# PaulMayer123/IMS-Toucan-Prosody-Variance

Hardware: AMD Instinct MI355X
Metric: mel-frames/sec + vocoder RTF @24kHz, batch=32, 1/2/4/8 MI355X (higher is better)
Workload: dtype bf16

## Files before the change

ims-toucan-prosody-variance_amd/csrc/common.h:

```cpp
#pragma once
#include <hip/hip_runtime.h>
#include <stdint.h>
#include <stdio.h>

#include "../../include/toucan_tts.h"

namespace tts {

void set_error(const char* fmt, ...);

#define TTS_CHECK_ARG(cond, ...)   \
  do {                             \
    if (!(cond)) {                 \
      tts::set_error(__VA_ARGS__); \
      return TTS_E_ARG;            \
    }                              \
  } while (0)

inline int launch_status(const char* what) {
  hipError_t e = hipGetLastError();
  if (e != hipSuccess) {
    set_error("%s: %s", what, hipGetErrorString(e));
    return TTS_E_LAUNCH;
  }
  return TTS_OK;
}

inline hipError_t raise_lds_limit(const void* kernel, unsigned long long& mask) {
  int dev = 0;
  (void)hipGetDevice(&dev);
  const unsigned long long bit = 1ull << (dev & 63);
  if (mask & bit) return hipSuccess;
  int room = 160 * 1024;
  hipFuncAttributes attr;
  if (hipFuncGetAttributes(&attr, kernel) == hipSuccess) room -= (int)attr.sharedSizeBytes;
  else (void)hipGetLastError();
  const hipError_t e = hipFuncSetAttribute(kernel, hipFuncAttributeMaxDynamicSharedMemorySize, room);
  if (e == hipSuccess) mask |= bit;
  else (void)hipGetLastError();
  return e;
}

struct WavenetCond {
  const float* g;
  int ld_g;
  const void* wc;
  int wc_n;
  int col0;
  const float* bc;
};
int wavenet_layer_cond(const TtsWavenetDesc& d, const WavenetCond& c, hipStream_t st);

typedef float f32x16 __attribute__((ext_vector_type(16)));
typedef float f32x4 __attribute__((ext_vector_type(4)));
typedef short bf16x8 __attribute__((ext_vector_type(8)));

__device__ __forceinline__ unsigned short f32_to_bf16(float f) {
  const __bf16 b = (__bf16)f;
  return __builtin_bit_cast(unsigned short, b);
}
__device__ __forceinline__ float bf16_to_f32(unsigned short u) { return __builtin_bit_cast(float, (unsigned int)u << 16); }

typedef _Float16 f16x2 __attribute__((ext_vector_type(2)));
typedef _Float16 f16x8 __attribute__((ext_vector_type(8)));
typedef float f32x2 __attribute__((ext_vector_type(2)));
__device__ __forceinline__ unsigned short f32_to_f16(float f) { return __builtin_bit_cast(unsigned short, (_Float16)f); }
__device__ __forceinline__ float f16_to_f32(unsigned short u) { return (float)__builtin_bit_cast(_Float16, u); }
template <bool F16>
__device__ __forceinline__ unsigned short to16(float f) {
  if constexpr (F16) return f32_to_f16(f);
  else return f32_to_bf16(f);
}
template <bool F16>
__device__ __forceinline__ float from16(unsigned short u) {
  if constexpr (F16) return f16_to_f32(u);
  else return bf16_to_f32(u);
}
template <bool F16>
__device__ __forceinline__ unsigned int pack16(float lo, float hi) {
  if constexpr (F16) {
    const f32x2 v = {lo, hi};
    return __builtin_bit_cast(unsigned int, __builtin_convertvector(v, f16x2));
  } else {
    return (unsigned int)f32_to_bf16(lo) | ((unsigned int)f32_to_bf16(hi) << 16);
  }
}
__device__ __forceinline__ float load16(unsigned short u, bool f16) { return f16 ? f16_to_f32(u) : bf16_to_f32(u); }
__device__ __forceinline__ unsigned short store16(float v, bool f16) { return f16 ? f32_to_f16(v) : f32_to_bf16(v); }

template <bool F16>
__device__ __forceinline__ f32x16 mfma16(bf16x8 a, bf16x8 b, f32x16 c) {
  if constexpr (F16) return __builtin_amdgcn_mfma_f32_32x32x16_f16(__builtin_bit_cast(f16x8, a), __builtin_bit_cast(f16x8, b), c, 0, 0, 0);
  else return __builtin_amdgcn_mfma_f32_32x32x16_bf16(a, b, c, 0, 0, 0);
}

#define TTS_GLOAD128(dst_, ptr_) asm volatile("global_load_dwordx4 %0, %1, off" : "=v"(dst_) : "v"(ptr_) : "memory")
#define TTS_GLOAD32(dst_, ptr_) asm volatile("global_load_dword %0, %1, off" : "=v"(dst_) : "v"(ptr_) : "memory")
#define TTS_WAIT_VM(n_) asm volatile("s_waitcnt vmcnt(%0)" ::"n"(n_) : "memory")
#define TTS_PIN(r_) asm volatile("" : "+v"(r_))

__device__ __forceinline__ float sigmoidf_(float v) { return 1.0f / (1.0f + __expf(-v)); }

__device__ __forceinline__ float wave_sum(float v) {
#pragma unroll
  for (int o = 32; o > 0; o >>= 1) v += __shfl_xor(v, o, 64);
  return v;
}

__device__ __forceinline__ float wave_max(float v) {
#pragma unroll
  for (int o = 32; o > 0; o >>= 1) v = fmaxf(v, __shfl_xor(v, o, 64));
  return v;
}

}
```

ims-toucan-prosody-variance_amd/csrc/conv1d_wide.hip:

```cpp
#include "common.h"
#include "conv_epilogue.h"

namespace tts {

namespace {

constexpr int WIDE_BM = 256, WIDE_BN = 256, WIDE_BK = 64, WIDE_THREADS = 512;
constexpr int WIDE_ROW_BYTES = WIDE_BK * 2;
constexpr int WIDE_SLAB_BYTES = WIDE_BK * WIDE_BN * 2;

__host__ __device__ inline int wide_win_rows(int taps, int dil) { return (WIDE_BM + (taps - 1) * dil + 7) & ~7; }
inline size_t wide_lds_bytes(int taps, int dil) {
  return (size_t)2 * wide_win_rows(taps, dil) * WIDE_ROW_BYTES + 2 * WIDE_SLAB_BYTES + 2 * WIDE_BN * sizeof(float);
}

__device__ __forceinline__ void wide_dma16(const void* src, void* lds_wave_base) {
  __builtin_amdgcn_global_load_lds((const void __attribute__((address_space(1)))*)src, (void __attribute__((address_space(3)))*)lds_wave_base, 16, 0, 0);
}

template <bool F16>
__global__ __launch_bounds__(WIDE_THREADS) void conv1d_wide_kernel(const TtsConvDesc d) {
  constexpr int TM = 4, TN = 2;
  extern __shared__ __attribute__((aligned(16))) unsigned char lds_raw[];

  const TtsTile tile = d.tiles[blockIdx.x];
  const int n0 = blockIdx.y * WIDE_BN;
  const int win_rows = wide_win_rows(d.taps, d.dil);
  const int win_bytes = win_rows * WIDE_ROW_BYTES;
  unsigned char* const xs0 = lds_raw;
  unsigned char* const ws0 = lds_raw + 2 * win_bytes;
  float* const eb = reinterpret_cast<float*>(ws0 + 2 * WIDE_SLAB_BYTES);

  const int tid = threadIdx.x;
  const int lane = tid & 63;
  const int wave = __builtin_amdgcn_readfirstlane(tid >> 6);
  const int wm = wave >> 2, wn = wave & 3;
  const int lrow = lane & 31, lk = lane >> 5;

  f32x16 acc[1][TM][TN];
#pragma unroll
  for (int i = 0; i < TM; ++i)
#pragma unroll
    for (int j = 0; j < TN; ++j)
#pragma unroll
      for (int r = 0; r < 16; ++r) acc[0][i][j][r] = 0.0f;

  if (tid < WIDE_BN) {
    const int n = n0 + tid;
    eb[tid] = (d.bias && n < d.cout) ? d.bias[n] : 0.0f;
    eb[WIDE_BN + tid] = 0.0f;
  }

  const bool poly = d.io_flags & TTS_IO_POLYPHASE;
  const int half = d.wn >> 1;
  const int tap_lo = (poly && n0 >= half) ? 1 : 0;
  const int tap_hi = (poly && n0 + WIDE_BN <= half) ? 2 : d.taps;
  const int wc0 = n0 + wn * 64;
  const int skip_tap = !poly ? -1 : (wc0 >= half ? 0 : (wc0 + 64 <= half ? 2 : -1));

  const int row_first = tile.row0 - d.pad_left;
  const bool edge = row_first < tile.seq_begin || row_first + win_rows > tile.seq_end;
  const unsigned short* __restrict__ xh = reinterpret_cast<const unsigned short*>(d.x);
  const unsigned short* __restrict__ W = reinterpret_cast<const unsigned short*>(d.w);
  const int n_chunks = d.cin / WIDE_BK;
  const int n_win_inst = win_rows >> 3;

  auto request_window = [&](int ch) __attribute__((always_inline)) {
    unsigned char* xb = xs0 + (ch & 1) * win_bytes;
    for (int i = wave; i < n_win_inst; i += 8) {
      const int wr = i * 8 + (lane >> 3);
      const int g = (lane & 7) ^ ((wr >> 1) & 7);
      const int gr = row_first + wr;
      const int grc = gr < tile.seq_begin ? tile.seq_begin : (gr >= tile.seq_end ? tile.seq_end - 1 : gr);
      wide_dma16(xh + (size_t)grc * d.ldx + ch * WIDE_BK + g * 8, xb + i * 1024);
    }
  };
  auto zero_window_edges = [&](int ch) __attribute__((always_inline)) {
    unsigned char* xb = xs0 + (ch & 1) * win_bytes;
    for (int i = wave; i < n_win_inst; i += 8) {
      const int gr = row_first + i * 8 + (lane >> 3);
      if (gr < tile.seq_begin || gr >= tile.seq_end) *reinterpret_cast<uint4*>(xb + i * 1024 + lane * 16) = make_uint4(0, 0, 0, 0);
    }
  };
  auto request_weights = [&](int ch, int tap, int buf) __attribute__((always_inline)) {
    unsigned char* wb = ws0 + buf * WIDE_SLAB_BYTES;
#pragma unroll
    for (int q = 0; q < 4; ++q) {
      const int idx = q * 8 + wave;
      const int kb = idx >> 2, part = idx & 3;
      const size_t goff = (((size_t)tap * (d.cin_pad >> 3) + ch * 8 + kb) * d.wn + n0 + part * 64 + lane) * 8;
      wide_dma16(W + goff, wb + idx * 1024);
    }
  };

  request_window(0);
  request_weights(0, tap_lo, 0);
  bool zero_pending = edge;
  int zero_ch = 0;

  int step = 0;
  for (int ch = 0; ch < n_chunks; ++ch) {
    const unsigned char* xb = xs0 + (ch & 1) * win_bytes;
    for (int tap = tap_lo; tap < tap_hi; ++tap, ++step) {
      asm volatile("s_waitcnt vmcnt(0)" ::: "memory");
      if (zero_pending) {
        zero_window_edges(zero_ch);
        zero_pending = false;
      }
      asm volatile("s_waitcnt lgkmcnt(0)\n\ts_barrier" ::: "memory");
      {
        const bool last_tap = tap + 1 == tap_hi;
        const int nch = last_tap ? ch + 1 : ch, ntap = last_tap ? tap_lo : tap + 1;
        if (nch < n_chunks) request_weights(nch, ntap, (step + 1) & 1);
      }
      if (tap == tap_lo && ch + 1 < n_chunks) {
        request_window(ch + 1);
        zero_pending = edge;
        zero_ch = ch + 1;
      }
      if (tap == skip_tap) continue;
      const unsigned char* wb = ws0 + (step & 1) * WIDE_SLAB_BYTES;
      const int r0 = wm * 128 + lrow + tap * d.dil;
#pragma unroll
      for (int ks = 0; ks < 4; ++ks) {
        const int g = ks * 2 + lk;
        bf16x8 a[TM], b[TN];
#pragma unroll
        for (int j = 0; j < TN; ++j) b[j] = *reinterpret_cast<const bf16x8*>(wb + (size_t)(g * WIDE_BN + wn * 64 + j * 32 + lrow) * 16);
#pragma unroll
        for (int i = 0; i < TM; ++i) {
          const int r = r0 + i * 32;
          a[i] = *reinterpret_cast<const bf16x8*>(xb + r * WIDE_ROW_BYTES + ((g ^ ((r >> 1) & 7)) << 4));
        }
#pragma unroll
        for (int i = 0; i < TM; ++i)
#pragma unroll
          for (int j = 0; j < TN; ++j) acc[0][i][j] = mfma16<F16>(b[j], a[i], acc[0][i][j]);
      }
    }
  }
  conv_epilogue_t<TM, TN, 1, false, true>(d, tile, n0, wm, wn, lrow, lk, acc, eb, WIDE_BN);
}

}

const char* conv1d_wide_reject(const TtsConvDesc& d) {
  auto al16 = [](const void* p) { return (reinterpret_cast<uintptr_t>(p) & 15) == 0; };
  if (d.compute != TTS_COMPUTE_BF16 && d.compute != TTS_COMPUTE_F16) return "compute must be bf16 or fp16";
  if (d.mode != TTS_MODE_LINEAR) return "mode must be LINEAR";
  if (!(d.io_flags & TTS_IO_X_BF16) || !(d.io_flags & TTS_IO_Y_BF16) || (d.res && !(d.io_flags & TTS_IO_RES_BF16))) return "x, y and res must be 16-bit tensors";
  if (((d.io_flags & TTS_IO_F16) != 0) != (d.compute == TTS_COMPUTE_F16)) return "the 16-bit tensors must be in the call's own format";
  if (d.pre_act != TTS_PRE_NONE) return "no pre-activation";
  if (d.seqvec || d.preadd || d.aux) return "no seqvec, preadd or aux";
  if (d.cin != d.cin_pad || d.cin % WIDE_BK != 0) return "cin must be unpadded and a multiple of 64";
  if (d.wn % WIDE_BN != 0 || d.cout > d.wn) return "wn must be a multiple of 256";
  if ((d.cout & 3) || (d.bias && !al16(d.bias))) return "cout must be a multiple of 4 and the bias 16-byte aligned";
  if ((d.ldx & 7) || (d.ldy & 7) || (d.res && (d.ld_res & 7)) || !al16(d.x) || !al16(d.y) || !al16(d.w) || (d.res && !al16(d.res))) return "rows and pointers must be 16-byte aligned";
  if ((d.io_flags & TTS_IO_POLYPHASE) && d.taps != 3) return "TTS_IO_POLYPHASE needs taps == 3";
  if (wide_lds_bytes(d.taps, d.dil) > 160 * 1024) return "the window does not fit in 160 KiB of LDS";
  return nullptr;
}

int conv1d_wide_launch(const TtsConvDesc& d, hipStream_t st) {
  const char* why = conv1d_wide_reject(d);
  TTS_CHECK_ARG(why == nullptr, "conv1d: a 256-row tile table asks for the wide tile, which this call cannot take: %s", why);
  const size_t lds = wide_lds_bytes(d.taps, d.dil);
  dim3 grid(d.n_tiles, d.wn / WIDE_BN), block(WIDE_THREADS);
  auto launch = [&](auto k, unsigned long long& raised) {
    if (lds > 64 * 1024) {
      const hipError_t e = raise_lds_limit(reinterpret_cast<const void*>(k), raised);
      if (e != hipSuccess) {
        set_error("conv1d (wide): raising the dynamic LDS limit failed: %s", hipGetErrorString(e));
        return (int)TTS_E_LAUNCH;
      }
    }
    hipLaunchKernelGGL(k, grid, block, lds, st, d);
    return launch_status("conv1d (wide)");
  };
  static unsigned long long raised_bf16 = 0, raised_f16 = 0;
  if (d.compute == TTS_COMPUTE_F16) return launch(conv1d_wide_kernel<true>, raised_f16);
  return launch(conv1d_wide_kernel<false>, raised_bf16);
}

}
```

ims-toucan-prosody-variance_amd/csrc/pipeline.hip:

```cpp
#include <algorithm>
#include <cmath>
#include <cstdlib>
#include <cstring>
#include <string>
#include <unordered_map>
#include <utility>
#include <vector>

#include "common.h"
#include "../../include/toucan_prosody.h"
#include "../../include/toucan_score.h"

namespace tts {

const char* conv1d_wide_reject(const TtsConvDesc& d);

namespace {

constexpr int ATT = 192, HEADS = 4, DK = 48;

struct Dev {
  void* p = nullptr;
  int64_t shape[4] = {0, 0, 0, 0};
  int ndim = 0, dtype = 0;
// ... 76 lines not shown
  }
  Layout halved() const {
    Layout l;
    for (size_t i = 0; i < begins.size(); ++i) {
      l.begins.push_back(begins[i] / 2);
      l.lengths.push_back(lengths[i] / 2);
      l.max_len = std::max(l.max_len, lengths[i] / 2);
    }
    l.total = total / 2;
    return l;
  }
  int n() const { return (int)lengths.size(); }
};

struct Arena {
  char* base = nullptr;
  size_t cap = 0, off = 0;
  void reset() { off = 0; }
};

struct TileTab {
  TtsTile* dev = nullptr;
  int n = 0;
};

constexpr size_t TABLE_FIRST_CHUNK = 64 << 10;
constexpr size_t TABLE_BUDGET = 16 << 20;

struct TableChunk {
  char* dev = nullptr;
  char* host = nullptr;
  size_t cap = 0, off = 0;
};

struct TableStore {
  std::vector<TableChunk> chunks;
  std::unordered_map<std::string, std::pair<void*, int>> index;
  hipEvent_t last_use = nullptr;
};

struct ProfRec {
  std::string name;
  double flops = 0, bytes = 0, elems = 0;
  hipEvent_t e0 = nullptr, e1 = nullptr;
};

}

struct Handle {
  TtsConfig cfg;
  std::unordered_map<std::string, Dev> weights;
  Acoustic acoustic;
  Vocoder vocoder;
  Arena phone, frame, voc[2];
  Arena nll;
  TableStore tabs[2][2];
  int tab_gen[2] = {0, 0};
  int tab_which = 0;
  long long n_tables_built = 0;
  int small_tile_blocks = 1536;
  int split_mode = 0;
  float* ptab[2] = {nullptr, nullptr};
  int pmax = 0;
  Layout lp, lf;
  int B = 0;
  const float* text = nullptr;
  float *e_norm = nullptr, *enc = nullptr, *pitch = nullptr, *energy = nullptr, *cln = nullptr;
  int* dur = nullptr;
  float *cat = nullptr, *dec = nullptr, *mel0 = nullptr, *mel = nullptr;
  std::vector<int> frames;
  float* pstats = nullptr;
  std::vector<float> pstats_host;
  bool have_flow = false;
  bool prof_on = false, prof_detail = false;
  std::string prof_select;
  std::vector<ProfRec> prof;
  std::vector<hipEvent_t> event_pool;
};

namespace {

#define TTS_TRY(expr)            \
  do {                           \
    const int rc_ = (expr);      \
    if (rc_ != TTS_OK) return rc_; \
  } while (0)

bool is16(const Handle* h);

#define TTS_CHECK_RESOLVED(h, entry) TTS_CHECK_ARG((h)->acoustic.resolved, entry ": weights were loaded since tts_encoder: run it again")

int hip_ok(hipError_t e, const char* what) {
  if (e == hipSuccess) return TTS_OK;
  set_error("%s: %s", what, hipGetErrorString(e));
  return TTS_E_LAUNCH;
}

int arena_reserve(Arena& a, size_t bytes, hipStream_t st) {
  a.reset();
  if (a.cap >= bytes) return TTS_OK;
  if (a.base) {
    TTS_TRY(hip_ok(hipStreamSynchronize(st), "workspace: stream sync before regrowth"));
    (void)hipFree(a.base);
    a.base = nullptr;
    a.cap = 0;
  }
  const size_t want = bytes + bytes / 8 + (1 << 20);
  TTS_TRY(hip_ok(hipMalloc(reinterpret_cast<void**>(&a.base), want), "workspace: hipMalloc"));
  a.cap = want;
  return TTS_OK;
}

template <class T>
T* arena_alloc(Arena& a, size_t count) {
  const size_t bytes = (count * sizeof(T) + 255) & ~(size_t)255;
  if (a.off + bytes > a.cap) return nullptr;
  T* p = reinterpret_cast<T*>(a.base + a.off);
  a.off += bytes;
  return p;
}

#define TTS_ALLOC(var, arena, T, count)                                                        \
  T* var = arena_alloc<T>(arena, (size_t)(count));                                             \
  if (!var) {                                                                                  \
    set_error("%s: workspace exhausted (%zu of %zu bytes used)", __func__, (arena).off, (arena).cap); \
    return TTS_E_ARG;                                                                          \
  }

std::string layout_key(const Layout& l, int tile_rows) {
  std::string k(reinterpret_cast<const char*>(l.begins.data()), l.begins.size() * sizeof(int));
  k.append(reinterpret_cast<const char*>(l.lengths.data()), l.lengths.size() * sizeof(int));
  k.append(reinterpret_cast<const char*>(&tile_rows), sizeof(int));
  return k;
}

int tables_begin(Handle* h, int which, hipStream_t st) {
  h->tab_which = which;
  h->tab_gen[which] ^= 1;
  TableStore& s = h->tabs[which][h->tab_gen[which]];
  if (!s.last_use) return TTS_OK;
  size_t held = 0;
  for (const TableChunk& c : s.chunks) held += c.off;
  if (held > TABLE_BUDGET) {
    TTS_TRY(hip_ok(hipEventSynchronize(s.last_use), "tile tables: last use before rewinding"));
    s.index.clear();
    for (TableChunk& c : s.chunks) c.off = 0;
    return TTS_OK;
  }
  const hipError_t q = hipEventQuery(s.last_use);
  if (q == hipSuccess) return TTS_OK;
  if (q != hipErrorNotReady) return hip_ok(q, "tile tables: last use");
  (void)hipGetLastError();
  return hip_ok(hipStreamWaitEvent(st, s.last_use, 0), "tile tables: wait for last use");
}

template <class Build>
int table_of(Handle* h, const std::string& key, hipStream_t st, Build build, void** dev, int* n) {
  TableStore& s = h->tabs[h->tab_which][h->tab_gen[h->tab_which]];
  auto it = s.index.find(key);
  if (it == s.index.end()) {
    auto host = build();
    const int count = (int)host.size();
    if (host.empty()) host.resize(1);
    const size_t bytes = host.size() * sizeof(host[0]), need = (bytes + 255) & ~(size_t)255;
    TableChunk* c = nullptr;
    for (TableChunk& k : s.chunks)
      if (k.off + need <= k.cap) {
        c = &k;
        break;
      }
    if (!c) {
      TableChunk k;
      k.cap = std::max(s.chunks.empty() ? TABLE_FIRST_CHUNK : 2 * s.chunks.back().cap, need);
      TTS_TRY(hip_ok(hipMalloc(reinterpret_cast<void**>(&k.dev), k.cap), "tile tables: hipMalloc"));
      const hipError_t e = hipHostMalloc(reinterpret_cast<void**>(&k.host), k.cap, hipHostMallocDefault);
      if (e != hipSuccess) (void)hipFree(k.dev);
      TTS_TRY(hip_ok(e, "tile tables: hipHostMalloc"));
      s.chunks.push_back(k);
      c = &s.chunks.back();
    }
    memcpy(c->host + c->off, host.data(), bytes);
    TTS_TRY(hip_ok(hipMemcpyAsync(c->dev + c->off, c->host + c->off, bytes, hipMemcpyHostToDevice, st), "tile tables: upload"));
    it = s.index.emplace(key, std::make_pair(static_cast<void*>(c->dev + c->off), count)).first;
    c->off += need;
    ++h->n_tables_built;
  }
  *dev = it->second.first;
  if (n) *n = it->second.second;
  return TTS_OK;
}

int tiles_of(Handle* h, const Layout& l, int tile_rows, hipStream_t st, TileTab* out) {
  void* dev;
  TTS_TRY(table_of(h, layout_key(l, tile_rows), st, [&] {
    std::vector<TtsTile> host;
    for (int u = 0; u < l.n(); ++u)
      for (int r = 0; r < l.lengths[u]; r += tile_rows) host.push_back(TtsTile{l.begins[u] + r, l.begins[u], l.begins[u] + l.lengths[u], u});
    return host;
  }, &dev, &out->n));
  out->dev = static_cast<TtsTile*>(dev);
  return TTS_OK;
}

int bounds_of(Handle* h, const Layout& l, hipStream_t st, const int** sb, const int** se) {
  void* dev;
  TTS_TRY(table_of(h, layout_key(l, -1), st, [&] {
    std::vector<int> host(2 * std::max(1, l.n()));
    for (int u = 0; u < l.n(); ++u) {
      host[u] = l.begins[u];
      host[l.n() + u] = l.begins[u] + l.lengths[u];
    }
    return host;
  }, &dev, nullptr));
  *sb = static_cast<const int*>(dev);
  *se = *sb + l.n();
  return TTS_OK;
}

const Dev* find(const Handle* h, const std::string& name) {
  auto it = h->weights.find(name);
  return it == h->weights.end() ? nullptr : &it->second;
}

int need(const Handle* h, const std::string& name, const Dev** out) {
  *out = find(h, name);
  if (!*out) {
    set_error("weight '%s' was not loaded (tts_load_weights)", name.c_str());
    return TTS_E_ARG;
  }
  return TTS_OK;
}

int fvec(const Handle* h, const std::string& name, const float** out) {
  const Dev* d;
  TTS_TRY(need(h, name, &d));
  *out = static_cast<const float*>(d->p);
  return TTS_OK;
}

int conv_of(const Handle* h, const std::string& name, ConvW* c) {
  const Dev *w, *m;
  TTS_TRY(need(h, name + ".w", &w));
  TTS_TRY(need(h, name + ".meta", &m));
  const int* mm = static_cast<const int*>(m->p);
  c->w = static_cast<const float*>(w->p);
  const Dev* w16 = find(h, name + ".w16");
  c->w16 = w16 ? w16->p : nullptr;
  const Dev* b = find(h, name + ".bias");
  c->bias = b ? static_cast<const float*>(b->p) : nullptr;
  c->mode = mm[0]; c->taps = mm[1]; c->dil = mm[2]; c->pad_left = mm[3]; c->cin = mm[4]; c->cin_pad = mm[5]; c->cout = mm[6];
  c->wn = mm[7]; c->half_pad = mm[8]; c->tile_rows = mm[9]; c->small_tile_rows = mm[10]; c->small_only = mm[11]; c->n_tile = mm[12];
  c->compute16 = mm[13];
  c->algo_taps = mm[14] > 0 ? mm[14] : c->taps;
  return TTS_OK;
}

hipEvent_t prof_event(Handle* h) {
  if (!h->event_pool.empty()) {
    hipEvent_t e = h->event_pool.back();
    h->event_pool.pop_back();
    return e;
  }
  hipEvent_t e = nullptr;
  (void)hipEventCreate(&e);
  return e;
}

template <class Launch>
int prof_launch(Handle* h, const char* name, double flops, double bytes, double elems, hipStream_t st, Launch launch) {
  if (!h->prof_on || !(h->prof_select.empty() || h->prof_select == name)) return launch();
  h->prof.emplace_back();
  ProfRec* r = &h->prof.back();
  r->name = name; r->flops = flops; r->bytes = bytes; r->elems = elems;
  r->e0 = prof_event(h);
  r->e1 = prof_event(h);
  (void)hipEventRecord(r->e0, st);
  const int rc = launch();
  (void)hipEventRecord(r->e1, st);
  return rc;
}

struct T2 {
  void* p;
  int ld;
  int bits;
  T2() : p(nullptr), ld(0), bits(32) {}
  T2(void* p_, int ld_, int bits_ = 32) : p(p_), ld(ld_), bits(bits_) {}
};

struct ConvOpt {
  int pre = TTS_PRE_NONE;
  float pre_slope = 0.f;
  int act = TTS_ACT_NONE;
  float alpha = 1.f;
  const float* seqvec = nullptr; int ld_seqvec = 0;
  const float* preadd = nullptr; int ld_preadd = 0;
  T2 res; float res_scale = 1.f;
  const float* aux = nullptr; int ld_aux = 0;
  bool accumulate = false;
  bool fp32_only = false;
  bool no_split_k = false;
  const float *snake_alpha = nullptr, *snake_beta = nullptr, *snake_filt = nullptr;
};

int device_cus() {
  static int cus[64] = {0};
  int dev = 0;
  (void)hipGetDevice(&dev);
  int& c = cus[dev & 63];
  if (c == 0 && (hipDeviceGetAttribute(&c, hipDeviceAttributeMultiprocessorCount, dev) != hipSuccess || c < 1)) {
    (void)hipGetLastError();
    c = 256;
  }
  return c;
}

int conv(Handle* h, const ConvW& cw, T2 x, T2 y, const Layout& l, hipStream_t st, const ConvOpt& o = ConvOpt()) {
  int tile_rows = cw.tile_rows;
  if (h->small_tile_blocks && cw.small_tile_rows && !cw.small_only) {
    const int cols = cw.mode == TTS_MODE_LINEAR ? cw.wn : cw.half_pad;
    const long long grid = (long long)((l.total + cw.tile_rows - 1) / cw.tile_rows) * (cols / cw.n_tile);
    if (grid < h->small_tile_blocks) tile_rows = cw.small_tile_rows;
  }
  TileTab tt;
  TTS_TRY(tiles_of(h, l, tile_rows, st, &tt));
  TtsConvDesc d;
  memset(&d, 0, sizeof(d));
  bool use16 = !o.fp32_only && h->cfg.precision != TTS_COMPUTE_F32 && cw.w16 != nullptr;
  if (use16 && cw.compute16 == TTS_COMPUTE_F32X3) {
    const int cols = cw.mode == TTS_MODE_LINEAR ? cw.wn : cw.half_pad;
    const bool small = (long long)tt.n * (tile_rows / 64) * ((cols + 63) / 64) <= 128;
    if (h->split_mode == 2 || (h->split_mode == 1 && small)) use16 = false;
  }
  d.x = static_cast<const float*>(x.p); d.ldx = x.ld; d.cin = cw.cin;
  d.w = use16 ? cw.w16 : cw.w; d.cin_pad = cw.cin_pad; d.wn = cw.wn; d.half_pad = cw.half_pad;
  d.bias = cw.bias;
  d.y = static_cast<float*>(y.p); d.ldy = y.ld; d.cout = cw.cout;
  d.taps = cw.taps; d.dil = cw.dil; d.pad_left = cw.pad_left;
  d.pre_act = o.pre; d.pre_slope = o.pre_slope;
  d.snake_alpha = o.snake_alpha; d.snake_beta = o.snake_beta; d.snake_filt = o.snake_filt;
  d.mode = cw.mode; d.act = o.act; d.alpha = o.alpha;
  d.seqvec = o.seqvec; d.ld_seqvec = o.ld_seqvec;
  d.preadd = o.preadd; d.ld_preadd = o.ld_preadd;
  d.res = static_cast<const float*>(o.res.p); d.ld_res = o.res.ld; d.res_scale = o.res_scale;
  d.aux = o.aux; d.ld_aux = o.ld_aux;
  d.accumulate = o.accumulate ? 1 : 0;
  d.compute = use16 ? cw.compute16 : TTS_COMPUTE_F32;
  const bool any16 = x.bits == 16 || y.bits == 16 || (o.res.p && o.res.bits == 16);
  d.io_flags = (x.bits == 16 ? TTS_IO_X_BF16 : 0) | (y.bits == 16 ? TTS_IO_Y_BF16 : 0) | ((o.res.p && o.res.bits == 16) ? TTS_IO_RES_BF16 : 0) |
               ((any16 && h->cfg.precision == TTS_COMPUTE_F16) ? TTS_IO_F16 : 0);
  if (h->split_mode && !o.no_split_k && !is16(h) && d.compute == TTS_COMPUTE_F32)
    d.io_flags |= h->split_mode == 2 ? TTS_IO_SPLIT_K_ALWAYS : TTS_IO_SPLIT_K;
  if (cw.algo_taps == 2 && cw.taps == 3) d.io_flags |= TTS_IO_POLYPHASE;
  const bool wide_pays = (cw.cin / 64) * cw.taps >= 28 || ((d.io_flags & TTS_IO_POLYPHASE) && cw.wn >= 512);
  if (cw.tile_rows != 256 && wide_pays && conv1d_wide_reject(d) == nullptr) {
    long long t256 = 0;
    for (int n : l.lengths) t256 += (n + 255) / 256;
    if (t256 * (cw.wn / 256) >= device_cus()) {
      tile_rows = 256;
      TTS_TRY(tiles_of(h, l, tile_rows, st, &tt));
    }
  }
  d.tiles = tt.dev; d.n_tiles = tt.n; d.tile_rows = tile_rows;
  if (h->prof_on) {
    const bool dual = cw.mode != TTS_MODE_LINEAR;
    const bool wide = tile_rows == 256 && cw.tile_rows != 256;
    const int bm = tile_rows != cw.tile_rows ? tile_rows : cw.tile_rows, bn = wide ? 256 : (tile_rows != cw.tile_rows ? 64 : cw.n_tile);
    char name[96];
    int nlen = snprintf(name, sizeof(name), "conv1d_%s<%dx%d%s>", d.compute == TTS_COMPUTE_F32 ? "f32" : (d.compute == TTS_COMPUTE_BF16 ? "bf16" : (d.compute == TTS_COMPUTE_F16 ? "f16" : "f32x3")),
                        bm, bn, dual ? ",dual" : "");
    if (h->prof_detail)
      snprintf(name + nlen, sizeof(name) - nlen, "[%dx%d k%d r%d]", cw.cin, cw.cout * (dual ? 2 : 1), cw.taps, l.total);
    double rows = 0;
    for (int n : l.lengths) rows += n;
    const double ctot = (double)cw.cout * (dual ? 2 : 1);
    return prof_launch(h, name, 2.0 * rows * cw.cin * ctot * cw.algo_taps,
                       rows * (cw.cin * (x.bits / 8.0) + cw.cout * (y.bits / 8.0)) + cw.taps * cw.cin * ctot * (d.compute == TTS_COMPUTE_F32 ? 4 : 2),
                       rows * cw.cout, st, [&] { return tts_conv1d(&d, st); });
  }
  return tts_conv1d(&d, st);
}

int block_of(const Handle* h, const std::string& p, Block* b) {
  static const char* ln[5] = {"norm_ff_macaron", "norm_mha", "norm_conv", "norm_ff", "norm_final"};
  for (int i = 0; i < 5; ++i) {
    TTS_TRY(fvec(h, p + ln[i] + ".g", &b->ln_g[i]));
    TTS_TRY(fvec(h, p + ln[i] + ".b", &b->ln_b[i]));
  }
  TTS_TRY(conv_of(h, p + "ffm.w1", &b->ffm1));
  TTS_TRY(conv_of(h, p + "ffm.w2", &b->ffm2));
  TTS_TRY(conv_of(h, p + "ff.w1", &b->ff1));
  TTS_TRY(conv_of(h, p + "ff.w2", &b->ff2));
  b->ffm_fused = find(h, p + "ffm.fused");
  b->ff_fused = find(h, p + "ff.fused");
  TTS_TRY(conv_of(h, p + "qkv", &b->qkv));
  TTS_TRY(conv_of(h, p + "out", &b->out));
  TTS_TRY(conv_of(h, p + "pos", &b->pos));
  TTS_TRY(conv_of(h, p + "pw1", &b->pw1));
  TTS_TRY(conv_of(h, p + "pw2", &b->pw2));
  TTS_TRY(fvec(h, p + "u", &b->u));
  TTS_TRY(fvec(h, p + "v", &b->v));
  TTS_TRY(fvec(h, p + "dw_w", &b->dw_w));
  TTS_TRY(fvec(h, p + "dw_b", &b->dw_b));
  return TTS_OK;
}

int predictor_of(const Handle* h, const std::string& p, int layers, int first_cln, Predictor* out) {
  out->layers = layers;
  out->first_cln = first_cln;
  for (int i = 0; i < layers; ++i) {
    TTS_TRY(conv_of(h, p + ".conv." + std::to_string(i), &out->conv[i]));
    if (h->cfg.multispeaker) continue;
    TTS_TRY(fvec(h, p + ".norm." + std::to_string(i) + ".g", &out->g[i]));
    TTS_TRY(fvec(h, p + ".norm." + std::to_string(i) + ".b", &out->b[i]));
  }
  return conv_of(h, p + ".lin", &out->lin);
}

int resolve_acoustic(Handle* h) {
  Acoustic& m = h->acoustic;
  if (m.resolved) return TTS_OK;
  TTS_TRY(conv_of(h, "embed0", &m.embed0));
  TTS_TRY(conv_of(h, "embed2", &m.embed2));
  const Dev* lang = find(h, "lang_table");
  m.lang_table = lang ? static_cast<const float*>(lang->p) : nullptr;
  for (int b = 0; b < 6; ++b) {
    TTS_TRY(block_of(h, "enc." + std::to_string(b) + ".", &m.enc[b]));
    TTS_TRY(block_of(h, "dec." + std::to_string(b) + ".", &m.dec[b]));
  }
  TTS_TRY(fvec(h, "out_norm.g", &m.out_norm_g));
  TTS_TRY(fvec(h, "out_norm.b", &m.out_norm_b));
  if (h->cfg.multispeaker) {
    TTS_TRY(conv_of(h, "hs_h", &m.hs_h));
    TTS_TRY(conv_of(h, "hs_e", &m.hs_e));
    const Dev* w;
    TTS_TRY(need(h, "cln_weights", &w));
    m.cln_weights = static_cast<const float*>(w->p);
    m.n_mlp = (int)(w->bytes / 4 / tts_cln_mlp_weight_floats(64, 256));
  }
  TTS_TRY(predictor_of(h, "pitch", 7, 0, &m.pitch));
  TTS_TRY(predictor_of(h, "energy", 2, 7, &m.energy));
  TTS_TRY(predictor_of(h, "duration", 3, 9, &m.duration));
  TTS_TRY(fvec(h, "pitch_w", &m.pitch_w));
  TTS_TRY(fvec(h, "pitch_b", &m.pitch_b));
  TTS_TRY(fvec(h, "energy_w", &m.energy_w));
  TTS_TRY(fvec(h, "energy_b", &m.energy_b));
  TTS_TRY(conv_of(h, "feat_out", &m.feat_out));
  for (int i = 0; i < 5; ++i) {
    const std::string p = "postnet." + std::to_string(i);
    TTS_TRY(conv_of(h, p + ".conv", &m.postnet[i].conv));
    TTS_TRY(fvec(h, p + ".g", &m.postnet[i].g));
    TTS_TRY(fvec(h, p + ".b", &m.postnet[i].b));
  }
  TTS_TRY(conv_of(h, "g_proj", &m.g_proj));
  for (int b = 0; b < 18; ++b) {
    const std::string p = "flow." + std::to_string(b) + ".";
    TTS_TRY(conv_of(h, p + "start", &m.flow[b].start));
    TTS_TRY(conv_of(h, p + "end", &m.flow[b].end));
    TTS_TRY(conv_of(h, p + "cond", &m.flow[b].cond));
    TTS_TRY(fvec(h, p + "winv", &m.flow[b].winv));
    TTS_TRY(fvec(h, p + "an_bias", &m.flow[b].an_bias));
    TTS_TRY(fvec(h, p + "an_logs", &m.flow[b].an_logs));
  }
  for (int g = 0; g < 5; ++g)
    for (int i = 0; i < 4; ++i) {
      const std::string p = "flowgrp." + std::to_string(g) + ".";
      TTS_TRY(conv_of(h, p + "inl." + std::to_string(i), &m.flowgrp[g].inl[i]));
      TTS_TRY(conv_of(h, p + "res_skip." + std::to_string(i), &m.flowgrp[g].res_skip[i]));
    }
  const Dev* logdet = find(h, "flow.logdet");
  m.scoring = logdet != nullptr;
  if (m.scoring) {
    TTS_CHECK_ARG(logdet->dtype == 3 && logdet->bytes == sizeof(double), "weight 'flow.logdet' is not one float64 as two int32 words of host metadata");
    memcpy(&m.flow_logdet, logdet->p, sizeof(double));
    for (int b = 0; b < 18; ++b) {
      const std::string p = "flow." + std::to_string(b) + ".";
      TTS_TRY(fvec(h, p + "wfwd", &m.flow_fwd[b].wfwd));
      TTS_TRY(conv_of(h, p + "end_ml", &m.flow_fwd[b].end_ml));
      const ConvW& e = m.flow_fwd[b].end_ml;
      TTS_CHECK_ARG(e.mode == TTS_MODE_LINEAR && e.cin == ATT && e.cout == 160 && e.taps == 1, "weight '%send_ml' is not a plain 1-tap 192 -> 160 conv", p.c_str());
    }
  }
  m.resolved = true;
  return TTS_OK;
}

int resolve_vocoder(Handle* h) {
  Vocoder& m = h->vocoder;
  if (m.resolved) return TTS_OK;
  const bool big = h->cfg.vocoder == 2;
  TTS_TRY(conv_of(h, "voc.pre", &m.pre));
  for (int i = 0; i < 4; ++i) {
    TTS_TRY(conv_of(h, "voc.ups." + std::to_string(i), &m.ups[i]));
    for (int j = 0; j < 3; ++j)
      for (int dd = 0; dd < 3; ++dd) {
        const std::string p = "voc.blk." + std::to_string(i) + "." + std::to_string(j) + "." + std::to_string(dd);
        auto& k = m.blk[i][j][dd];
        TTS_TRY(conv_of(h, p + ".c1", &k.c1));
        TTS_TRY(conv_of(h, p + ".c2", &k.c2));
        if (!big) continue;
        TTS_TRY(fvec(h, p + ".a1", &k.a1));
        TTS_TRY(fvec(h, p + ".b1", &k.b1));
        TTS_TRY(fvec(h, p + ".a2", &k.a2));
        TTS_TRY(fvec(h, p + ".b2", &k.b2));
      }
  }
  TTS_TRY(fvec(h, "voc.post_w", &m.post_w));
  if (big) {
    TTS_TRY(fvec(h, "voc.post_a", &m.post_a));
    TTS_TRY(fvec(h, "voc.post_b", &m.post_b));
    TTS_TRY(fvec(h, "voc.filt", &m.filt));
    const Dev* ft;
    TTS_TRY(need(h, "voc.fir_tab", &ft));
    m.fir_tab = ft->p;
  }
  m.resolved = true;
  return TTS_OK;
}

bool is16(const Handle* h) { return h->cfg.precision == TTS_COMPUTE_BF16 || h->cfg.precision == TTS_COMPUTE_F16; }
int bits16(const Handle* h) { return is16(h) ? 16 : 32; }
bool postflow_cond_buffer(const Handle* h) { return !is16(h); }

int ensure_ptabs(Handle* h, hipStream_t st) {
  const Dev* pe;
  TTS_TRY(need(h, "pe", &pe));
  const int rows = (int)pe->shape[0], pmax = (rows + 1) / 2;
  if (h->pmax == pmax && h->ptab[0]) return TTS_OK;
  TTS_TRY(hip_ok(hipStreamSynchronize(st), "position tables: sync"));
  for (int s = 0; s < 2; ++s) {
    if (h->ptab[s]) (void)hipFree(h->ptab[s]);
    TTS_TRY(hip_ok(hipMalloc(reinterpret_cast<void**>(&h->ptab[s]), (size_t)6 * rows * ATT * sizeof(float)), "position tables: hipMalloc"));
  }
  int one = rows;
  const Layout l = Layout::make(&one, 1, 1);
  for (int s = 0; s < 2; ++s)
    for (int b = 0; b < 6; ++b) {
      ConvOpt o;
      o.fp32_only = true;
      o.no_split_k = true;
      TTS_TRY(conv(h, (s ? h->acoustic.dec : h->acoustic.enc)[b].pos, T2(pe->p, ATT), T2(h->ptab[s] + (size_t)b * rows * ATT, ATT), l, st, o));
    }
  h->pmax = pmax;
  return TTS_OK;
}

int ffn_fused(Handle* h, const Dev* fused, const ConvW& w1, const ConvW& w2, const float* g, const float* b, const float* post_g, const float* post_b,
              float* x, int R, hipStream_t st) {
  TtsFfnDesc d;
  memset(&d, 0, sizeof(d));
  d.x = x; d.ldx = ATT; d.y = x; d.ldy = ATT; d.rows = R; d.channels = ATT;
  d.ln_g = g; d.ln_b = b;
  d.w = fused->p; d.b2 = w2.bias;
  d.post_g = post_g; d.post_b = post_b;
  d.hidden = (int)(fused->bytes / (28 * 1024)) * 32;
  d.compute = w1.compute16; d.alpha = 0.5f; d.eps = 1e-12f;
  return prof_launch(h, d.compute == TTS_COMPUTE_F16 ? "ffn_fused_f16" : "ffn_fused_bf16", 4.0 * R * ATT * d.hidden,
                     (double)R * ATT * 8 + (double)fused->bytes, (double)R * ATT, st, [&] { return tts_ffn_fused(&d, st); });
}

int conformer(Handle* h, int stack, float* x, const Layout& l, Arena& a, hipStream_t st) {
  const int R = l.total, kernel = stack ? 31 : 7;
  if (l.max_len > h->pmax) {
    set_error("conformer: %d positions exceed the uploaded position table (pmax %d): upload a larger 'pe'", l.max_len, h->pmax);
    return TTS_E_ARG;
  }
  const int b16 = bits16(h);
  TTS_ALLOC(ln, a, float, (size_t)R * ATT);
  TTS_ALLOC(hid, a, char, (size_t)R * 1536 * (b16 / 8));
  TTS_ALLOC(qkv, a, float, (size_t)R * 3 * ATT);
  TTS_ALLOC(ctx, a, float, (size_t)R * ATT);
  TTS_ALLOC(glu, a, float, (size_t)R * ATT);
  TTS_ALLOC(dwo, a, float, (size_t)R * ATT);
  TileTab t128, t64;
  TTS_TRY(tiles_of(h, l, 128, st, &t128));
  TTS_TRY(tiles_of(h, l, 64, st, &t64));
  const size_t prow = (size_t)(2 * h->pmax - 1) * ATT;
  for (int bi = 0; bi < 6; ++bi) {
    const Block& b = (stack ? h->acoustic.dec : h->acoustic.enc)[bi];
    ConvOpt relu, half, res1;
    relu.act = TTS_ACT_RELU;
    half.alpha = 0.5f; half.res = T2(x, ATT);
    res1.res = T2(x, ATT);
    const bool fuse_ffn = b16 == 16;
    if (fuse_ffn && b.ffm_fused) {
      TTS_TRY(ffn_fused(h, b.ffm_fused, b.ffm1, b.ffm2, b.ln_g[0], b.ln_b[0], nullptr, nullptr, x, R, st));
    } else {
      TTS_TRY(tts_layernorm(x, ATT, ln, ATT, b.ln_g[0], b.ln_b[0], R, ATT, 1e-12f, st));
      TTS_TRY(conv(h, b.ffm1, T2(ln, ATT), T2(hid, 1536, b16), l, st, relu));
      TTS_TRY(conv(h, b.ffm2, T2(hid, 1536, b16), T2(x, ATT), l, st, half));
    }
    TTS_TRY(tts_layernorm(x, ATT, ln, ATT, b.ln_g[1], b.ln_b[1], R, ATT, 1e-12f, st));
    TTS_TRY(conv(h, b.qkv, T2(ln, ATT), T2(qkv, 3 * ATT), l, st));
    if (b16 == 16)
      TTS_TRY(tts_relpos_attention_f16(qkv, 3 * ATT, h->ptab[stack] + bi * prow, h->pmax, b.u, b.v, ctx, ATT, HEADS, DK, t128.dev, t128.n, 128, st));
    else
      TTS_TRY(tts_relpos_attention(qkv, 3 * ATT, h->ptab[stack] + bi * prow, h->pmax, b.u, b.v, ctx, ATT, HEADS, DK, t128.dev, t128.n, 128,
                                   h->split_mode == 2 ? TTS_ATT_KEY_SPLIT_ALWAYS : (h->split_mode == 1 ? TTS_ATT_KEY_SPLIT : 0), st));
    TTS_TRY(conv(h, b.out, T2(ctx, ATT), T2(x, ATT), l, st, res1));
    TTS_TRY(tts_layernorm(x, ATT, ln, ATT, b.ln_g[2], b.ln_b[2], R, ATT, 1e-12f, st));
    TTS_TRY(conv(h, b.pw1, T2(ln, ATT), T2(glu, ATT), l, st));
    TTS_TRY(tts_dwconv_swish(glu, ATT, dwo, ATT, b.dw_w, b.dw_b, ATT, kernel, t64.dev, t64.n, 64, st));
    TTS_TRY(conv(h, b.pw2, T2(dwo, ATT), T2(x, ATT), l, st, res1));
    if (fuse_ffn && b.ff_fused) {
      TTS_TRY(ffn_fused(h, b.ff_fused, b.ff1, b.ff2, b.ln_g[3], b.ln_b[3], b.ln_g[4], b.ln_b[4], x, R, st));
    } else {
      TTS_TRY(tts_layernorm(x, ATT, ln, ATT, b.ln_g[3], b.ln_b[3], R, ATT, 1e-12f, st));
      TTS_TRY(conv(h, b.ff1, T2(ln, ATT), T2(hid, 1536, b16), l, st, relu));
      TTS_TRY(conv(h, b.ff2, T2(hid, 1536, b16), T2(x, ATT), l, st, half));
      TTS_TRY(tts_layernorm(x, ATT, x, ATT, b.ln_g[4], b.ln_b[4], R, ATT, 1e-12f, st));
    }
  }
  return TTS_OK;
}

size_t conformer_bytes(size_t R) { return R * (ATT * 4 * 4 + 1536 * 4 + 3 * ATT * 4) + 8 * 256; }

size_t phone_arena_bytes(size_t R, size_t B) {
// ... 894 lines not shown
```

Measured before the change: 588,700.

## Split tail-wave wide conv tiles into half-width tiles to balance CUs

The wide conv kernel now runs on a 1D grid. When the last wave of 256x256 workgroups would fill at most half the CUs, those leftover tiles are each split into two 256x128 workgroups, so more CUs share the tail. The tile body is templated on column width, with the wave layout and TM adjusted to match. This aims to cut tail-wave idle time in exchange for some redundant input-window loads and smaller, less efficient tiles at the tail.

```diff
diff --git a/ims-toucan-prosody-variance_amd/csrc/common.h b/ims-toucan-prosody-variance_amd/csrc/common.h
--- a/ims-toucan-prosody-variance_amd/csrc/common.h
+++ b/ims-toucan-prosody-variance_amd/csrc/common.h
@@ -39,6 +39,18 @@
   if (e == hipSuccess) mask |= bit;
   else (void)hipGetLastError();
   return e;
+}
+
+inline int device_cus() {
+  static int cus[64] = {0};
+  int dev = 0;
+  (void)hipGetDevice(&dev);
+  int& c = cus[dev & 63];
+  if (c == 0 && (hipDeviceGetAttribute(&c, hipDeviceAttributeMultiprocessorCount, dev) != hipSuccess || c < 1)) {
+    (void)hipGetLastError();
+    c = 256;
+  }
+  return c;
 }
 
 struct WavenetCond {
diff --git a/ims-toucan-prosody-variance_amd/csrc/conv1d_wide.hip b/ims-toucan-prosody-variance_amd/csrc/conv1d_wide.hip
--- a/ims-toucan-prosody-variance_amd/csrc/conv1d_wide.hip
+++ b/ims-toucan-prosody-variance_amd/csrc/conv1d_wide.hip
@@ -18,13 +18,12 @@
   __builtin_amdgcn_global_load_lds((const void __attribute__((address_space(1)))*)src, (void __attribute__((address_space(3)))*)lds_wave_base, 16, 0, 0);
 }
 
-template <bool F16>
-__global__ __launch_bounds__(WIDE_THREADS) void conv1d_wide_kernel(const TtsConvDesc d) {
-  constexpr int TM = 4, TN = 2;
-  extern __shared__ __attribute__((aligned(16))) unsigned char lds_raw[];
-
-  const TtsTile tile = d.tiles[blockIdx.x];
-  const int n0 = blockIdx.y * WIDE_BN;
+template <bool F16, int BN>
+__device__ __forceinline__ void wide_tile(const TtsConvDesc& d, const TtsTile tile, const int n0, unsigned char* const lds_raw) {
+  constexpr int WN_WAVES = BN / 64, WM_WAVES = 8 / WN_WAVES;
+  constexpr int TM = WIDE_BM / (WM_WAVES * 32), TN = 2;
+  constexpr int SLAB_BYTES = WIDE_BK * BN * 2;
+
   const int win_rows = wide_win_rows(d.taps, d.dil);
   const int win_bytes = win_rows * WIDE_ROW_BYTES;
   unsigned char* const xs0 = lds_raw;
@@ -34,7 +33,7 @@
   const int tid = threadIdx.x;
   const int lane = tid & 63;
   const int wave = __builtin_amdgcn_readfirstlane(tid >> 6);
-  const int wm = wave >> 2, wn = wave & 3;
+  const int wm = wave / WN_WAVES, wn = wave % WN_WAVES;
   const int lrow = lane & 31, lk = lane >> 5;
 
   f32x16 acc[1][TM][TN];
@@ -45,16 +44,16 @@
 #pragma unroll
       for (int r = 0; r < 16; ++r) acc[0][i][j][r] = 0.0f;
 
-  if (tid < WIDE_BN) {
+  if (tid < BN) {
     const int n = n0 + tid;
     eb[tid] = (d.bias && n < d.cout) ? d.bias[n] : 0.0f;
-    eb[WIDE_BN + tid] = 0.0f;
+    eb[BN + tid] = 0.0f;
   }
 
   const bool poly = d.io_flags & TTS_IO_POLYPHASE;
   const int half = d.wn >> 1;
   const int tap_lo = (poly && n0 >= half) ? 1 : 0;
-  const int tap_hi = (poly && n0 + WIDE_BN <= half) ? 2 : d.taps;
+  const int tap_hi = (poly && n0 + BN <= half) ? 2 : d.taps;
   const int wc0 = n0 + wn * 64;
   const int skip_tap = !poly ? -1 : (wc0 >= half ? 0 : (wc0 + 64 <= half ? 2 : -1));
 
@@ -83,11 +82,11 @@
     }
   };
   auto request_weights = [&](int ch, int tap, int buf) __attribute__((always_inline)) {
-    unsigned char* wb = ws0 + buf * WIDE_SLAB_BYTES;
-#pragma unroll
-    for (int q = 0; q < 4; ++q) {
+    unsigned char* wb = ws0 + buf * SLAB_BYTES;
+#pragma unroll
+    for (int q = 0; q < WN_WAVES; ++q) {
       const int idx = q * 8 + wave;
-      const int kb = idx >> 2, part = idx & 3;
+      const int kb = idx / WN_WAVES, part = idx % WN_WAVES;
       const size_t goff = (((size_t)tap * (d.cin_pad >> 3) + ch * 8 + kb) * d.wn + n0 + part * 64 + lane) * 8;
       wide_dma16(W + goff, wb + idx * 1024);
     }
@@ -119,14 +118,14 @@
         zero_ch = ch + 1;
       }
       if (tap == skip_tap) continue;
-      const unsigned char* wb = ws0 + (step & 1) * WIDE_SLAB_BYTES;
-      const int r0 = wm * 128 + lrow + tap * d.dil;
+      const unsigned char* wb = ws0 + (step & 1) * SLAB_BYTES;
+      const int r0 = wm * (TM * 32) + lrow + tap * d.dil;
 #pragma unroll
       for (int ks = 0; ks < 4; ++ks) {
         const int g = ks * 2 + lk;
         bf16x8 a[TM], b[TN];
 #pragma unroll
-        for (int j = 0; j < TN; ++j) b[j] = *reinterpret_cast<const bf16x8*>(wb + (size_t)(g * WIDE_BN + wn * 64 + j * 32 + lrow) * 16);
+        for (int j = 0; j < TN; ++j) b[j] = *reinterpret_cast<const bf16x8*>(wb + (size_t)(g * BN + wn * 64 + j * 32 + lrow) * 16);
 #pragma unroll
         for (int i = 0; i < TM; ++i) {
           const int r = r0 + i * 32;
@@ -139,7 +138,19 @@
       }
     }
   }
-  conv_epilogue_t<TM, TN, 1, false, true>(d, tile, n0, wm, wn, lrow, lk, acc, eb, WIDE_BN);
+  conv_epilogue_t<TM, TN, 1, false, true>(d, tile, n0, wm, wn, lrow, lk, acc, eb, BN);
+}
+
+template <bool F16>
+__global__ __launch_bounds__(WIDE_THREADS) void conv1d_wide_kernel(const TtsConvDesc d, const int n_full) {
+  extern __shared__ __attribute__((aligned(16))) unsigned char lds_raw[];
+  const int b = blockIdx.x;
+  if (b < n_full) {
+    wide_tile<F16, WIDE_BN>(d, d.tiles[b % d.n_tiles], (b / d.n_tiles) * WIDE_BN, lds_raw);
+  } else {
+    const int h = b - n_full, pair = n_full + (h >> 1);
+    wide_tile<F16, WIDE_BN / 2>(d, d.tiles[pair % d.n_tiles], (pair / d.n_tiles) * WIDE_BN + (h & 1) * (WIDE_BN / 2), lds_raw);
+  }
 }
 
 }
@@ -161,11 +172,19 @@
   return nullptr;
 }
 
+static int wide_full_pairs(long long n_wg, int cus) {
+  const long long rem = n_wg % cus;
+  return (int)((rem > 0 && rem <= cus / 2) ? n_wg - rem : n_wg);
+}
+
 int conv1d_wide_launch(const TtsConvDesc& d, hipStream_t st) {
   const char* why = conv1d_wide_reject(d);
   TTS_CHECK_ARG(why == nullptr, "conv1d: a 256-row tile table asks for the wide tile, which this call cannot take: %s", why);
   const size_t lds = wide_lds_bytes(d.taps, d.dil);
-  dim3 grid(d.n_tiles, d.wn / WIDE_BN), block(WIDE_THREADS);
+  const long long n_wg = (long long)d.n_tiles * (d.wn / WIDE_BN);
+  TTS_CHECK_ARG(n_wg < (1ll << 30), "conv1d (wide): %lld workgroups are too many for one launch", n_wg);
+  const int n_full = wide_full_pairs(n_wg, device_cus());
+  dim3 grid((unsigned)(n_full + 2 * (n_wg - n_full))), block(WIDE_THREADS);
   auto launch = [&](auto k, unsigned long long& raised) {
     if (lds > 64 * 1024) {
       const hipError_t e = raise_lds_limit(reinterpret_cast<const void*>(k), raised);
@@ -174,7 +193,7 @@
         return (int)TTS_E_LAUNCH;
       }
     }
-    hipLaunchKernelGGL(k, grid, block, lds, st, d);
+    hipLaunchKernelGGL(k, grid, block, lds, st, d, n_full);
     return launch_status("conv1d (wide)");
   };
   static unsigned long long raised_bf16 = 0, raised_f16 = 0;
diff --git a/ims-toucan-prosody-variance_amd/csrc/pipeline.hip b/ims-toucan-prosody-variance_amd/csrc/pipeline.hip
--- a/ims-toucan-prosody-variance_amd/csrc/pipeline.hip
+++ b/ims-toucan-prosody-variance_amd/csrc/pipeline.hip
@@ -402,18 +402,6 @@
   bool no_split_k = false;
   const float *snake_alpha = nullptr, *snake_beta = nullptr, *snake_filt = nullptr;
 };
-
-int device_cus() {
-  static int cus[64] = {0};
-  int dev = 0;
-  (void)hipGetDevice(&dev);
-  int& c = cus[dev & 63];
-  if (c == 0 && (hipDeviceGetAttribute(&c, hipDeviceAttributeMultiprocessorCount, dev) != hipSuccess || c < 1)) {
-    (void)hipGetLastError();
-    c = 256;
-  }
-  return c;
-}
 
 int conv(Handle* h, const ConvW& cw, T2 x, T2 y, const Layout& l, hipStream_t st, const ConvOpt& o = ConvOpt()) {
   int tile_rows = cw.tile_rows;
```

Result: no change. 588,000 (median of 2 runs) (-0.1%).
